# minio/minlz

Hardware: AMD Instinct MI355X
Metric: MB/s encode+decode, 8MB blocks L1 (higher is better)
Workload: dtype u8; 1 GPU; enwik8-like synthetic text (the reference's L1 compresses it to ~0.47; enwik8 itself is not available offline), 100000000 B per GPU in 8 MiB blocks (12 blocks), level 1, far=1; step = encode all blocks + decode all blocks, HBM-resident; block_size=8388608, bytes_per_gpu=100000000, ranks=1, backend=none (single process), device=AMD Radeon Graphics (gfx950:sramecc+:xnack-)

## Files before the change

minlz_amd/csrc/mlz_encode.hip.inc:

```

namespace mlz {

constexpr uint32_t kLaneCap = 32;
#ifndef MLZ_FAR_BITS
#define MLZ_FAR_BITS 17
#endif
#ifndef MLZ_EPOCH_LOG
#define MLZ_EPOCH_LOG 21
#endif
constexpr int kFarBits = MLZ_FAR_BITS;
constexpr int kEpochLog = MLZ_EPOCH_LOG;
static_assert((1u << kEpochLog) <= kMaxCopy3Offset, "a position's own epoch lies within one copy3 offset");
constexpr int kFarStride = 4;
#ifndef MLZ_SMALL_FB_SHIFT
#define MLZ_SMALL_FB_SHIFT 2
#endif
__host__ __device__ __forceinline__ constexpr int small_far_bits(uint64_t block_len) {
    int lg = 14 + MLZ_SMALL_FB_SHIFT;
    while (lg < 17 + MLZ_SMALL_FB_SHIFT && (1ull << lg) < block_len) lg++;
    return lg - MLZ_SMALL_FB_SHIFT;
}
constexpr uint32_t kFarMin = 8;
constexpr int kLevels = 4;

__device__ __forceinline__ uint64_t ld64u(const uint8_t* p) {
    uint64_t v;
    __builtin_memcpy(&v, p, 8);
    return v;
}
constexpr int kFarTagBits = 9;
constexpr uint32_t kFarTagMask = (1u << kFarTagBits) - 1;
struct FarHash { uint32_t idx, tag; };
__device__ __forceinline__ FarHash far_hash(uint64_t v, int bits, uint32_t tagmask = kFarTagMask) {
    const uint32_t a = (uint32_t(v) * 0x9E3779B1u + uint32_t(v >> 32)) * 0x85EBCA77u;
    return {a >> (32 - bits), (a >> (32 - bits - kFarTagBits)) & tagmask};
}
__device__ __forceinline__ uint32_t ctz64(uint64_t v) { return __builtin_ctzll(v); }
__device__ __forceinline__ uint64_t ballot64(bool p) { return __ballot(p); }
__device__ __forceinline__ uint32_t rdlane(uint32_t v, int l) { return __builtin_amdgcn_readlane(v, l); }
__device__ __forceinline__ uint32_t rdfirst(uint32_t v) { return __builtin_amdgcn_readfirstlane(v); }

constexpr uint32_t kPatternFast = 0xE4E4E4E4u;
#ifndef MLZ_PATTERN_DENSE
#define MLZ_PATTERN_DENSE 0xEEE7B9E4u
#endif
constexpr uint32_t kPatternDense = MLZ_PATTERN_DENSE;
#ifndef MLZ_PATTERN_THREE
#define MLZ_PATTERN_THREE 0xA9A9A994u
#endif
constexpr uint32_t kPatternThree = MLZ_PATTERN_THREE;
constexpr uint32_t kPatternFree = 0u;
__host__ __device__ __forceinline__ int tile_level_p(uint32_t tile_in_block, uint32_t pattern) { return int((pattern >> (2 * (tile_in_block & 15))) & 3); }
__host__ __device__ __forceinline__ int tile_level(uint32_t tile_in_block) { return tile_level_p(tile_in_block, kPatternFast); }
__host__ __device__ __forceinline__ uint32_t level_pattern_of(int level) { return level >= 2 ? kPatternDense : kPatternThree; }

__host__ __device__ __forceinline__ uint32_t far_sets(uint32_t pattern) { return pattern == kPatternFree ? 1u : uint32_t(kLevels - 1); }

__device__ __forceinline__ uint32_t match_len(const uint8_t* a, const uint8_t* b, uint32_t max) {
    uint32_t n = 0;
    while (n + 8 <= max) {
        uint64_t d = ld64u(a + n) ^ ld64u(b + n);
        if (d) return n + (ctz64(d) >> 3);
        n += 8;
    }
    while (n < max && a[n] == b[n]) n++;
    return n;
}

constexpr int kFarSliceBits = 15;
constexpr int kL2FarBitsBig = 18;
__host__ __device__ constexpr uint32_t far_tag_mask(int FB) { return FB == kL2FarBitsBig ? 0x1E0u : kFarTagMask; }
constexpr uint32_t far_slices(int fb) { return 1u << (fb - kFarSliceBits); }
constexpr uint64_t kBigBlock = 1u << 20;
template <int FB, int ST>
__global__ __launch_bounds__(1024) void far_build_kernel(const uint8_t* __restrict__ src_base, const BlockInfo* __restrict__ blocks,
                                                         uint32_t* __restrict__ far_tab, uint32_t epochs_per_block, uint32_t pattern,
                                                         uint32_t tab_log, uint32_t cls) {
    extern __shared__ __attribute__((aligned(16))) uint8_t smem[];
    uint32_t* slot = reinterpret_cast<uint32_t*>(smem);
    const uint32_t slice = blockIdx.x;
    const uint32_t ep = blockIdx.y;
    const BlockInfo b = blocks[blockIdx.z];
    if (cls != 2 && uint32_t(b.src_len >= kBigBlock) != cls) return;
    if (b.src_len > kMaxBlockSize) return;
    const int fb = FB ? FB : small_far_bits(b.src_len) + (ST == 2 ? 1 : 0);
    const uint32_t tlog = FB ? uint32_t(FB) : tab_log;
    const int sbits = fb < kFarSliceBits ? fb : kFarSliceBits;
    if (slice >= (1u << (fb - sbits))) return;
    const uint8_t* s = src_base + b.src_off;
    const int tid = threadIdx.x;
    for (uint32_t i = tid; i < (1u << sbits) / 4; i += 1024) reinterpret_cast<uint4*>(slot)[i] = uint4{0xffffffffu, 0xffffffffu, 0xffffffffu, 0xffffffffu};
    __syncthreads();
    const uint64_t e0 = uint64_t(ep) << kEpochLog;
    const uint64_t e1 = e0 + (1ull << kEpochLog) < b.src_len ? e0 + (1ull << kEpochLog) : b.src_len;
    constexpr uint32_t kPerTile = kTile / ST / 1024;
    constexpr int kFbTiles = ST >= 4 ? 2 : 1;
    constexpr uint32_t kBatch = kFbTiles * kPerTile;
    const uint32_t tiles_in_epoch = e1 > e0 && b.src_len >= 8 ? uint32_t((e1 - e0 + kTile - 1) >> kTileLog) : 0;
    constexpr uint32_t kEpochTiles = 1u << (kEpochLog - kTileLog);
    static_assert(kEpochTiles % 64 == 0, "an epoch is a whole number of 64-tile groups (4 periods of the level pattern each)");
    uint32_t need = 0;
    const bool free_levels = pattern == kPatternFree;
    {
        const uint64_t nt = (b.src_len + kTile - 1) >> kTileLog;
        for (uint32_t k = 1; k < 16 && k < nt; k++) need = need > uint32_t(tile_level_p(k, pattern)) ? need : uint32_t(tile_level_p(k, pattern));
        if (free_levels) need = nt > 1 ? 1 : 0;
    }
    for (uint32_t lset = 0; lset < need; lset++) {
      for (uint32_t g64 = 0; g64 < kEpochTiles; g64 += 64) {
        const uint32_t left = tiles_in_epoch > g64 ? tiles_in_epoch - g64 : 0;
        const uint64_t in_epoch = left >= 64 ? ~0ull : ((1ull << left) - 1);
        uint64_t todo = 0;
        for (uint32_t k = 0; k < 16; k++)
            if (free_levels || uint32_t(tile_level_p(k, pattern)) == lset) todo |= 0x0001000100010001ull << k;
        todo &= in_epoch;
        while (todo) {
            uint32_t kk[kFbTiles];
#pragma unroll
            for (int t = 0; t < kFbTiles; t++) { kk[t] = todo ? g64 + uint32_t(ctz64(todo)) : tiles_in_epoch; todo &= todo - 1; }
            uint64_t w[kBatch];
            uint64_t qq[kBatch];
            bool ok[kBatch];
#pragma unroll
            for (uint32_t u = 0; u < kBatch; u++) {
                const uint32_t k = kk[u / kPerTile];
                const uint64_t q = e0 + (uint64_t(k) << kTileLog) + (uint64_t(u % kPerTile) * 1024 + tid) * ST;
                qq[u] = q;
                ok[u] = k < tiles_in_epoch && q + 8 <= b.src_len && q < e1;
                w[u] = ld64u(s + (ok[u] ? q : 0));
            }
#pragma unroll
            for (uint32_t u = 0; u < kBatch; u++) {
                const FarHash fh = far_hash(w[u], fb, far_tag_mask(FB));
                if (ok[u] && (fh.idx >> sbits) == slice)
                    atomicMin(&slot[fh.idx & ((1u << sbits) - 1)], (uint32_t(qq[u]) << kFarTagBits) | fh.tag);
            }
        }
      }
        __syncthreads();
        const size_t tab = ((size_t(blockIdx.z) * far_sets(pattern) + lset) * epochs_per_block + ep) << tlog;
        uint32_t* out = far_tab + tab + (size_t(slice) << sbits);
        for (uint32_t i = tid; i < (1u << sbits) / 4; i += 1024) reinterpret_cast<uint4*>(out)[i] = reinterpret_cast<const uint4*>(slot)[i];
        __syncthreads();
    }
}

__device__ __forceinline__ uint32_t wave_incl_scan_u32(uint32_t v);
constexpr int kBinSliceBits = 14;
template <int FB, int ST> struct FarBin {
    static_assert(FB == kL2FarBitsBig, "the sorted word: 4 tag bits << 28 | window << 14 | bucket");
    static constexpr uint32_t kPerUnit = kTile / 2 / ST;
    static constexpr uint32_t kSlices = 1u << (FB - kBinSliceBits);
    static constexpr uint32_t kOffs = kSlices + 1;
    static constexpr uint32_t kCounters = 4 * kSlices * 64;
    static constexpr uint32_t kLds = kPerUnit * 4 + kCounters * 4 + kOffs * 4 + 64;
};
template <int FB, int ST>
__global__ __launch_bounds__(256) void far_bin_kernel(const uint8_t* __restrict__ src_base, const BlockInfo* __restrict__ blocks,
                                                      const uint32_t* __restrict__ tile_block, uint32_t* __restrict__ bins,
                                                      uint32_t* __restrict__ binoff) {
    using C = FarBin<FB, ST>;
    constexpr uint32_t kPerUnit = C::kPerUnit, kPerWave = kPerUnit / 4, kRounds = kPerWave / 64, kS = C::kSlices;
    static_assert(kPerUnit <= (1u << 14) && kRounds <= 64 && kRounds % 16 == 0, "window index in 14 bits; a lane's words in registers");
    extern __shared__ __attribute__((aligned(16))) uint8_t smem[];
    uint32_t* B = reinterpret_cast<uint32_t*>(smem);
    uint32_t* cnt = B + kPerUnit;
    uint32_t* segoff = cnt + C::kCounters;
    uint32_t* wsum = segoff + C::kOffs;
    const uint32_t unit = blockIdx.x, gt = unit >> 1;
    const BlockInfo b = blocks[tile_block[gt]];
    if (b.src_len < kBigBlock) return;
    const uint32_t tib = gt - b.first_tile;
    const uint64_t base = (uint64_t(tib) << kTileLog) + (unit & 1) * (kTile / 2);
    const uint8_t* s = src_base + b.src_off;
    const int tid = threadIdx.x, lane = tid & 63;
    const uint32_t wv = rdfirst(uint32_t(tid) >> 6);
    for (uint32_t i = tid; i < C::kCounters / 4; i += 256) reinterpret_cast<uint4*>(cnt)[i] = uint4{0, 0, 0, 0};
    __syncthreads();
    uint32_t word[kRounds];
    uint8_t tag4[kRounds];
    uint32_t* mine = cnt + wv * 64 + lane;
#pragma unroll
    for (uint32_t r0 = 0; r0 < kRounds; r0 += 16) {
        uint64_t w[16];
        bool ok[16];
#pragma unroll
        for (int u = 0; u < 16; u++) {
            const uint64_t q = base + uint64_t(wv * kPerWave + (r0 + u) * 64 + lane) * ST;
            ok[u] = q + 8 <= b.src_len;
            w[u] = ld64u(s + (ok[u] ? q : 0));
        }
#pragma unroll
        for (int u = 0; u < 16; u++) {
            const FarHash fh = far_hash(w[u], FB, far_tag_mask(FB));
            const uint32_t j = wv * kPerWave + (r0 + u) * 64 + lane;
            word[r0 + u] = ok[u] ? (fh.idx >> kBinSliceBits) << 28 | j << kBinSliceBits | (fh.idx & ((1u << kBinSliceBits) - 1)) : 0xffffffffu;
            tag4[r0 + u] = uint8_t(fh.tag >> 5);
            if (ok[u]) atomicAdd(&mine[(fh.idx >> kBinSliceBits) * 256], 1u);
        }
    }
    __syncthreads();
    {
        uint32_t v[16], sum = 0;
#pragma unroll
        for (int i = 0; i < 16; i++) { v[i] = cnt[tid * 16 + i]; sum += v[i]; }
        const uint32_t incl = wave_incl_scan_u32(sum);
        if (lane == 63) wsum[wv] = incl;
        __syncthreads();
        uint32_t carry = 0;
#pragma unroll
        for (uint32_t k = 0; k < 4; k++) carry += k < wv ? wsum[k] : 0;
        uint32_t run = carry + incl - sum;
#pragma unroll
        for (int i = 0; i < 16; i++) { cnt[tid * 16 + i] = run; run += v[i]; }
        if (tid == 255) segoff[kS] = run;
        __syncthreads();
        if (tid < int(kS)) segoff[tid] = cnt[tid * 256];
    }
#pragma unroll
    for (uint32_t r = 0; r < kRounds; r++)
        if (word[r] != 0xffffffffu) B[atomicAdd(&mine[(word[r] >> 28) * 256], 1u)] = (word[r] & 0x0fffffffu) | uint32_t(tag4[r]) << 28;
    __syncthreads();
    const uint32_t total = segoff[kS];
    uint32_t* out = bins + size_t(unit) * kPerUnit;
    for (uint32_t i = tid * 4; i < total; i += 1024) reinterpret_cast<uint4*>(out + i)[0] = reinterpret_cast<const uint4*>(B + i)[0];
    if (tid < int(C::kOffs)) binoff[size_t(unit) * C::kOffs + tid] = segoff[tid];
}

template <int FB, int ST>
__global__ __launch_bounds__(1024) void far_slice_kernel(const BlockInfo* __restrict__ blocks, const uint32_t* __restrict__ bins,
                                                         const uint32_t* __restrict__ binoff, uint32_t* __restrict__ far_tab, uint32_t epochs_per_block) {
    using C = FarBin<FB, ST>;
    constexpr uint32_t kPerUnit = C::kPerUnit, kSlice = 1u << kBinSliceBits;
    constexpr uint32_t kEpochUnits = 2u << (kEpochLog - kTileLog);
    static_assert(kEpochUnits == 128, "128 half tiles per epoch: a thread pair per unit for the segment offsets");
    extern __shared__ __attribute__((aligned(16))) uint8_t smem[];
    uint32_t* slot = reinterpret_cast<uint32_t*>(smem);
    uint32_t* so = slot + kSlice;
    const uint32_t slice = blockIdx.x, ep = blockIdx.y;
    const BlockInfo b = blocks[blockIdx.z];
    if (b.src_len < kBigBlock || b.n_tiles == 0) return;
    const uint32_t units_len = uint32_t((b.src_len + kTile / 2 - 1) / (kTile / 2));
    const uint32_t units = units_len < 2 * b.n_tiles ? units_len : 2 * b.n_tiles;
    const uint32_t u0 = ep * kEpochUnits, u1 = u0 + kEpochUnits < units ? u0 + kEpochUnits : units;
    if (u0 >= u1) return;
    const uint32_t nu = u1 - u0;
    const size_t unit0 = size_t(b.first_tile) * 2 + u0;
    const int tid = threadIdx.x;
    if (tid < 256) {
        const uint32_t u = uint32_t(tid) >> 1;
        so[tid] = u < nu ? binoff[(unit0 + u) * C::kOffs + slice + (tid & 1)] : 0u;
    }
    for (uint32_t i = tid; i < kSlice / 4; i += 1024) reinterpret_cast<uint4*>(slot)[i] = uint4{0xffffffffu, 0xffffffffu, 0xffffffffu, 0xffffffffu};
    __syncthreads();
    uint32_t* pre = so + 256;
    if (tid < 64) {
        const uint32_t a0 = so[4 * tid + 1] - so[4 * tid], a1 = so[4 * tid + 3] - so[4 * tid + 2];
        const uint32_t incl = wave_incl_scan_u32(a0 + a1);
        pre[2 * tid] = incl - a0 - a1; pre[2 * tid + 1] = incl - a1;
        if (tid == 63) pre[128] = incl;
    }
    __syncthreads();
    const uint32_t total = pre[128];
    for (uint32_t e0 = 0; e0 < total; e0 += 16 * 1024) {
        uint32_t w[16], ub[16];
#pragma unroll
        for (uint32_t k = 0; k < 16; k++) {
            const uint32_t e = e0 + 1024 * k + uint32_t(tid);
            const uint32_t ee = e < total ? e : total - 1;
            uint32_t u = 0;
#pragma unroll
            for (uint32_t step = 64; step; step >>= 1) u += pre[u + step] <= ee ? step : 0;
            ub[k] = e < total ? (u0 + u) * (kTile / 2) : 0xffffffffu;
            w[k] = bins[(unit0 + u) * kPerUnit + so[2 * u] + (ee - pre[u])];
        }
#pragma unroll
        for (uint32_t k = 0; k < 16; k++)
            if (ub[k] != 0xffffffffu)
                atomicMin(&slot[w[k] & (kSlice - 1)], (ub[k] + ((w[k] >> kBinSliceBits) & (kSlice - 1)) * ST) << kFarTagBits | (w[k] >> 28) << 5);
    }
    __syncthreads();
    uint32_t* tab = far_tab + ((size_t(blockIdx.z) * far_sets(kPatternFree) * epochs_per_block + ep) << FB) + (size_t(slice) << kBinSliceBits);
    for (uint32_t i = tid; i < kSlice / 4; i += 1024) reinterpret_cast<uint4*>(tab)[i] = reinterpret_cast<const uint4*>(slot)[i];
}

__device__ __forceinline__ uint64_t lds_ld64(const uint32_t* w, uint32_t p) {
    const uint32_t i = p >> 2, sh = p & 3;
    const uint32_t a = w[i], b = w[i + 1], c = w[i + 2];
    const uint32_t lo = __builtin_amdgcn_alignbyte(b, a, sh);
    const uint32_t hi = __builtin_amdgcn_alignbyte(c, b, sh);
    return lo | (uint64_t(hi) << 32);
}
__device__ __forceinline__ uint8_t lds_ld8(const uint32_t* w, uint32_t p) { return reinterpret_cast<const uint8_t*>(w)[p]; }
// ... 183 lines not shown
```

minlz_amd/csrc/mlz_hip.hip:

```cpp
#include <hip/hip_runtime.h>

#include <algorithm>
#include <atomic>
#include <condition_variable>
#include <cstdio>
#include <cstring>
#include <mutex>
#include <string>
#include <thread>
#include <type_traits>
#include <vector>

#include "../../include/minlz_hip.h"
#include "../../include/minlz_hip_search_batch.h"
#include "../../include/minlz_hip_search_batch_prune.h"
#include "../../include/minlz_hip_stream_set.h"
#include "../../include/minlz_hip_search_compressed.h"
#include "../../include/minlz_hip_search_compress.h"
#include "../../include/minlz_hip_sidecar_extract.h"
#include "../../include/minlz_hip_record_index_store.h"
#include "../../include/minlz_hip_encode_batch_tables.h"
#include "mlz_format.h"
#include "mlz_kernels.h"

// ... 165 lines not shown
        ev_res[id]++;
    }
};

namespace {

#define HIPCHK(ctx, call)                                                                 \
    do {                                                                                  \
        hipError_t e_ = (call);                                                           \
        if (e_ != hipSuccess) {                                                           \
            (ctx)->err = std::string(#call) + ": " + hipGetErrorString(e_);               \
            return -MLZ_ERR_HIP;                                                          \
        }                                                                                 \
    } while (0)

struct Timer {
    mlz_ctx* c; int id; hipStream_t s;
    bool on;
    Timer(mlz_ctx* c_, int id_, hipStream_t s_) : c(c_), id(id_), s(s_), on(c_->timing != 0 && ((c_->timer_mask >> id_) & 1) != 0) {
        if (!on) return;
        if (c->ev_last_call[id] != c->call_seq) {
            c->ev_last_call[id] = c->call_seq;
            if (c->timing == 1) {
                while (c->ev_res[id] < c->ev_cnt[id]) c->resolve_one(id);
                c->acc_ms[id] = 0; c->ev_calls[id] = 0;
            }
            c->ev_calls[id]++;
        }
        while (c->ev_cnt[id] - c->ev_res[id] >= uint64_t(mlz_ctx::kTimerRing)) c->resolve_one(id);
        (void)hipEventRecord(c->evr[id][c->ev_cnt[id] % mlz_ctx::kTimerRing][0], s);
    }
    ~Timer() {
        if (!on) return;
        (void)hipEventRecord(c->evr[id][c->ev_cnt[id] % mlz_ctx::kTimerRing][1], s);
        c->ev_cnt[id]++;
    }
};

struct WorkspaceOrder {
    mlz_ctx* c; hipStream_t s;
    WorkspaceOrder(mlz_ctx* c_, hipStream_t s_) : c(c_), s(s_) {
        if (c->ws_used && (c->ws_recorded || c->ws_stream != s)) {
            if (c->ws_recorded) (void)hipStreamWaitEvent(s, c->ws_done, 0);
            else if (hipEventRecord(c->ws_done, c->ws_stream) == hipSuccess) (void)hipStreamWaitEvent(s, c->ws_done, 0);
            else { (void)hipGetLastError(); (void)hipDeviceSynchronize(); }
        }
    }
    ~WorkspaceOrder() {
        c->ws_stream = s;
        c->ws_used = true;
        c->ws_recorded = false;
    }
};

int upload_blocks(mlz_ctx* c, hipStream_t st, const mlz_block_desc* desc, int n, bool tiles_from_dst, uint32_t* total_tiles, uint32_t* total_segs = nullptr,
                  const uint64_t* mirror = nullptr, bool any_length = false ) {
    c->dk = tiles_from_dst ? 1 : 0;
    std::vector<BlockInfo>& prev = c->h_blocks_prev_k[c->dk];
    c->h_blocks.resize(n);
    uint32_t tiles = 0, segs = 0;
    for (int i = 0; i < n; i++) {
        BlockInfo& b = c->h_blocks[i];
        b.src_off = desc[i].src_off; b.src_len = desc[i].src_len; b.dst_off = desc[i].dst_off; b.dst_cap = desc[i].dst_cap;
        b.mirror = mirror ? mirror[i] : 0;
        uint64_t span = tiles_from_dst ? desc[i].dst_cap : desc[i].src_len;
        if (span > kMaxBlockSize && !any_length) span = tiles_from_dst ? kMaxBlockSize : 0;
        b.first_tile = tiles;
        b.n_tiles = uint32_t((span + kTile - 1) >> kTileLog);
        tiles += b.n_tiles;
        b.first_seg = segs;
        b.n_segs = 0;
        if (tiles_from_dst) {
            uint64_t cl = std::min<uint64_t>(desc[i].src_len, 2 * std::min<uint64_t>(desc[i].dst_cap, kMaxBlockSize) + 32);
            b.n_segs = uint32_t((cl + kSeg - 1) >> kSegLog);
            segs += b.n_segs;
        }
    }
    *total_tiles = tiles;
    if (total_segs) *total_segs = segs;
    const bool same = prev.size() == c->h_blocks.size() && std::memcmp(prev.data(), c->h_blocks.data(), sizeof(BlockInfo) * n) == 0;
    if (same) return 0;
    c->h_tile_block.resize(tiles);
    c->h_seg_block.resize(segs);
    for (int i = 0; i < n; i++) {
        for (uint32_t t = 0; t < c->h_blocks[i].n_tiles; t++) c->h_tile_block[c->h_blocks[i].first_tile + t] = uint32_t(i);
        for (uint32_t t = 0; t < c->h_blocks[i].n_segs; t++) c->h_seg_block[c->h_blocks[i].first_seg + t] = uint32_t(i);
    }
    const size_t nb = sizeof(BlockInfo) * n, nt = sizeof(uint32_t) * tiles, ns = sizeof(uint32_t) * segs;
    const int sl = (c->up_slot ^= 1);
    if (c->upload_pending_k[sl]) { HIPCHK(c, hipEventSynchronize(c->upload_done_k[sl])); c->upload_pending_k[sl] = false; }
    if (nb + nt + ns > c->pinned_cap_k[sl]) {
        if (c->pinned_k[sl]) HIPCHK(c, hipHostFree(c->pinned_k[sl]));
        c->pinned_k[sl] = nullptr;
        c->pinned_cap_k[sl] = (nb + nt + ns) * 2 + 4096;
        HIPCHK(c, hipHostMalloc(&c->pinned_k[sl], c->pinned_cap_k[sl], hipHostMallocDefault));
    }
    char* pin = static_cast<char*>(c->pinned_k[sl]);
    HIPCHK(c, c->d_blocks_cur().ensure(nb + 64));
    HIPCHK(c, c->d_tile_block_cur().ensure(nt + 64));
    HIPCHK(c, c->d_seg_block_cur().ensure(ns + 64));
    std::memcpy(pin, c->h_blocks.data(), nb);
    std::memcpy(pin + nb, c->h_tile_block.data(), nt);
    std::memcpy(pin + nb + nt, c->h_seg_block.data(), ns);
    if (nb) HIPCHK(c, hipMemcpyAsync(c->d_blocks_cur().p, pin, nb, hipMemcpyHostToDevice, st));
    if (nt) HIPCHK(c, hipMemcpyAsync(c->d_tile_block_cur().p, pin + nb, nt, hipMemcpyHostToDevice, st));
    if (ns) HIPCHK(c, hipMemcpyAsync(c->d_seg_block_cur().p, pin + nb + nt, ns, hipMemcpyHostToDevice, st));
    HIPCHK(c, hipEventRecord(c->upload_done_k[sl], st));
    c->upload_pending_k[sl] = true;
    prev = c->h_blocks;
    return 0;
}

template <class F> int for_each_group(mlz_ctx* c, const mlz_block_desc* desc, int n, bool by_dst, F fn) {
    int b0 = 0;
    while (b0 < n) {
        uint64_t bytes = 0;
        int b1 = b0;
        while (b1 < n) {
            const uint64_t span = std::min<uint64_t>(by_dst ? desc[b1].dst_cap : desc[b1].src_len, kMaxBlockSize);
            if (b1 > b0 && bytes + span > c->device_group) break;
            bytes += span;
            b1++;
        }
        const int r = fn(b0, b1 - b0);
        if (r) return r;
        b0 = b1;
    }
    return 0;
}

template <class List> int raise_lds_once(mlz_ctx* c, bool& raised, const List& list) {
    if (raised) return 0;
    for (const auto& k : list) HIPCHK(c, hipFuncSetAttribute(reinterpret_cast<const void*>(k.fn), hipFuncAttributeMaxDynamicSharedMemorySize, int(k.lds)));
    raised = true;
    return 0;
}
template <class Fn> struct Kernel { Fn fn; uint32_t lds; };
struct AnyKernel : Kernel<const void*> { template <class F> AnyKernel(F* f, uint32_t l) : Kernel{reinterpret_cast<const void*>(f), l} {} };
using Kernels = std::initializer_list<AnyKernel>;

using MatchFn = void (*)(const uint8_t*, const BlockInfo*, const uint32_t*, uint2*, uint32_t*, const uint32_t*, uint32_t, uint32_t, uint32_t, uint32_t, uint32_t,
                         uint32_t, uint8_t*, uint32_t*);
enum MatchId { M_L1_BIG_FAR, M_L1_SMALL_FAR, M_L1_BIG, M_L1_SMALL, M_SUPERFAST, M_L2_BIG, M_L2_SMALL, M_L2_ONE_TILE, M_COUNT };
const Kernel<MatchFn> kMatch[M_COUNT] = {
    {match_tiles_kernel<true, MLZ_M2_NW, kM2HashBitsBig, kFarBits, false>, M2Cfg<kM2HashBitsBig>::kLds},
    {match_tiles_kernel<true, MLZ_M2_NW, kM2HashBitsSmall, 0, false>, M2Cfg<kM2HashBitsSmall>::kLds},
    {match_tiles_kernel<false, MLZ_M2_NW, kM2HashBitsBig, kFarBits, false>, M2Cfg<kM2HashBitsBig>::kLds},
    {match_tiles_kernel<false, MLZ_M2_NW, kM2HashBitsSmall, kFarBits, false>, M2Cfg<kM2HashBitsSmall>::kLds},
    {match_tiles_kernel<false, MLZ_M2_NW, kM2HashBitsSuperFast, kFarBits, false>, M2Cfg<kM2HashBitsSuperFast>::kLds},
    {match_tiles_kernel<true, MLZ_M2_NW, kM2HashBitsSmall, kL2FarBits, true>, M2Cfg<kM2HashBitsSmall>::kLds},
    {match_tiles_kernel<true, MLZ_M2_NW, kM2HashBitsSmall, 0, true>, M2Cfg<kM2HashBitsSmall>::kLds},
    {match_tiles_kernel<false, MLZ_M2_NW, kM2HashBitsSmall, kL2FarBits, true>, M2Cfg<kM2HashBitsSmall>::kLds},
};
using FarBuildFn = void (*)(const uint8_t*, const BlockInfo*, uint32_t*, uint32_t, uint32_t, uint32_t, uint32_t);
const Kernel<FarBuildFn> kFarBuild[4] = {
    {far_build_kernel<0, kFarStride>, 4u << kFarSliceBits}, {far_build_kernel<kFarBits, kFarStride>, 4u << kFarSliceBits},
    {far_build_kernel<0, kL2FarStride>, 4u << kFarSliceBits}, {far_build_kernel<kL2FarBits, kL2FarStride>, 4u << kFarSliceBits},
};

struct MatchPlan { int n; struct { MatchId id; uint32_t cls; } launch[2]; };
MatchPlan match_plan(int level, bool far, bool any_big, bool any_small) {
    if (level == MLZ_LEVEL_SUPERFAST) return {1, {{M_SUPERFAST, 2u}}};
    const bool l2 = level == MLZ_LEVEL_BALANCED;
    if (l2 && !far) return {1, {{M_L2_ONE_TILE, 2u}}};
    MatchPlan p{};
    if (any_big) p.launch[p.n++] = {l2 ? M_L2_BIG : far ? M_L1_BIG_FAR : M_L1_BIG, any_small ? 1u : 2u};
    if (any_small) p.launch[p.n++] = {l2 ? M_L2_SMALL : far ? M_L1_SMALL_FAR : M_L1_SMALL, any_big ? 0u : 2u};
    return p;
}

struct EncGroup {
    int level, n;
    const BlockInfo* blocks; const uint32_t* tile_block;
    uint32_t tiles, epochs, pattern, far_gap;
    size_t units;
    bool far, any_big, any_small;
    int fbits;
};

int encode_far_tables(mlz_ctx* c, hipStream_t st, const EncGroup& g, const uint8_t* d_src, const mlz_block_desc* desc) {
    Timer t(c, T_FAR, st);
    const bool l2 = g.level == MLZ_LEVEL_BALANCED;
    HIPCHK(c, c->d_far.ensure(((size_t(g.n) * far_sets(g.pattern) * g.epochs) << g.fbits) * 4));
    if (int r = raise_lds_once(c, c->far_attr, kFarBuild)) return r;
    auto build = [&](const Kernel<FarBuildFn>& v, dim3 grid, uint32_t lds, uint32_t cls) {
        hipLaunchKernelGGL(v.fn, grid, dim3(1024), lds, st, d_src, g.blocks, c->d_far.as<uint32_t>(), g.epochs, g.pattern, uint32_t(g.fbits), cls);
    };
    if (g.any_big) {
        if (l2 && g.pattern == kPatternFree && !c->far_slices_l2) {
            using FBn = FarBin<kL2FarBits, kL2FarStride>;
            const size_t units2 = size_t(g.tiles) * 2;
            HIPCHK(c, c->d_farbin.ensure(units2 * FBn::kPerUnit * 4 + units2 * FBn::kOffs * 4 + 256));
            uint32_t* bins = c->d_farbin.as<uint32_t>();
            uint32_t* binoff = bins + units2 * FBn::kPerUnit;
            constexpr uint32_t kSliceLds = (4u << kBinSliceBits) + 256 * 4 + 132 * 4;
            if (int r = raise_lds_once(c, c->farbin_attr, Kernels{{far_bin_kernel<kL2FarBits, kL2FarStride>, FBn::kLds}, {far_slice_kernel<kL2FarBits, kL2FarStride>, kSliceLds}})) return r;
            hipLaunchKernelGGL((far_bin_kernel<kL2FarBits, kL2FarStride>), dim3(uint32_t(units2)), dim3(256), FBn::kLds, st, d_src, g.blocks, g.tile_block, bins, binoff);
            hipLaunchKernelGGL((far_slice_kernel<kL2FarBits, kL2FarStride>), dim3(FBn::kSlices, g.epochs, g.n), dim3(1024), kSliceLds, st, g.blocks, bins, binoff, c->d_far.as<uint32_t>(), g.epochs);
        } else
            build(kFarBuild[2 * l2 + 1], dim3(far_slices(l2 ? kL2FarBits : kFarBits), g.epochs, g.n), kFarBuild[2 * l2 + 1].lds, g.any_small ? 1u : 2u);
    }
    if (g.any_small) {
        uint64_t max_small = 0;
        for (int i = 0; i < g.n; i++) if (desc[i].src_len < kBigBlock) max_small = std::max<uint64_t>(max_small, desc[i].src_len);
        const int sb = small_far_bits(max_small) + (l2 ? 1 : 0);
        const uint32_t lds = 4u << std::min<int>(sb, kFarSliceBits);
        build(kFarBuild[2 * l2], dim3(1u << (std::max<int>(sb, kFarSliceBits) - kFarSliceBits), 1, g.n), lds, g.any_big ? 0u : 2u);
    }
    return 0;
}

int encode_match(mlz_ctx* c, hipStream_t st, const EncGroup& g, const uint8_t* d_src) {
    HIPCHK(c, c->d_recs.ensure(g.units * kRecPerPiece * sizeof(uint2)));
    HIPCHK(c, c->d_piece_cnt.ensure(g.units * sizeof(uint32_t)));
    if (int r = raise_lds_once(c, c->enc_attrs, kMatch)) return r;
    const uint32_t* ftab = g.far ? c->d_far.as<uint32_t>() : nullptr;
    uint8_t* fuse_scratch = c->fuse_ser ? c->d_scratch.as<uint8_t>() : nullptr;
    {
        Timer t(c, T_ENC_TILES, st);
        const uint32_t grid = ((g.tiles + 7) / 8) * 8;
        const MatchPlan plan = match_plan(g.level, g.far, g.any_big, g.any_small);
        for (int i = 0; i < plan.n; i++) {
            const Kernel<MatchFn>& v = kMatch[plan.launch[i].id];
            hipLaunchKernelGGL(v.fn, dim3(grid), dim3(256), v.lds, st, d_src, g.blocks, g.tile_block, c->d_recs.as<uint2>(), c->d_piece_cnt.as<uint32_t>(), ftab, g.epochs,
                               g.pattern, g.tiles, plan.launch[i].cls, uint32_t(g.fbits), g.far_gap, fuse_scratch, c->d_tile_size.as<uint32_t>());
        }
    }
    if (!fuse_scratch) {
        Timer t(c, T_ENC_SER, st);
        hipLaunchKernelGGL(serialize_pieces_kernel, dim3(g.tiles), dim3(256), kSerLds, st, d_src, g.blocks, g.tile_block, c->d_recs.as<uint2>(),
                           c->d_piece_cnt.as<uint32_t>(), c->d_scratch.as<uint8_t>(), c->d_tile_size.as<uint32_t>());
    }
    return 0;
}

void encode_layout_gather(mlz_ctx* c, hipStream_t st, const EncGroup& g, const uint8_t* d_src, uint8_t* d_dst, const mlz_block_desc* desc, int64_t* d_out_len,
                          bool with_header) {
    bool fold = c->fold_layout && g.tiles > 0 && g.level != MLZ_LEVEL_UNCOMPRESSED;
    for (int i = 0; fold && i < g.n; i++) {
        const uint64_t len = desc[i].src_len;
        if (len == 0 || len > kMaxBlockSize || desc[i].dst_cap < (with_header ? len + 2 : len)) fold = false;
    }
    if (!fold) {
        Timer t(c, T_ENC_LAYOUT, st);
        hipLaunchKernelGGL(encode_layout_kernel, dim3(g.n), dim3(64), 0, st, g.blocks, c->d_tile_size.as<uint32_t>(), c->d_tile_out.as<uint32_t>(), d_dst, d_out_len,
                           c->d_flags.as<uint32_t>(), g.level, with_header ? 1 : 0, kSubLog);
    }
    if (g.tiles > 0) {
        Timer t(c, T_ENC_GATHER, st);
        const auto gather = fold ? encode_gather2_kernel<true> : encode_gather2_kernel<false>;
        hipLaunchKernelGGL(gather, dim3(g.tiles), dim3(256), 0, st, d_src, g.blocks, g.tile_block, c->d_scratch.as<uint8_t>(),
                           c->d_tile_size.as<uint32_t>(), c->d_tile_out.as<uint32_t>(), d_dst, c->d_flags.as<uint32_t>(), with_header ? 1 : 0, g.level, d_out_len);
    }
}

int encode_device_group(mlz_ctx* c, hipStream_t st, int level, const uint8_t* d_src, uint8_t* d_dst, const mlz_block_desc* desc, int n,
                        int64_t* d_out_len, bool with_header, const uint64_t* mirror) {
    EncGroup g{level, n};
    int r = upload_blocks(c, st, desc, n, false, &g.tiles, nullptr, mirror);
    if (r) return r;
    g.blocks = c->d_blocks_cur().as<BlockInfo>(); g.tile_block = c->d_tile_block_cur().as<uint32_t>();
    g.units = size_t(g.tiles) << kSubLog;
    HIPCHK(c, c->d_tile_size.ensure(sizeof(uint32_t) * (g.units + 1)));
    HIPCHK(c, c->d_tile_out.ensure(sizeof(uint32_t) * (g.units + 1)));
    HIPCHK(c, c->d_flags.ensure(sizeof(uint32_t) * n));
    if (level != MLZ_LEVEL_UNCOMPRESSED && g.tiles > 0) {
        HIPCHK(c, c->d_scratch.ensure(g.units * kPieceScratch));
        const bool l2 = level == MLZ_LEVEL_BALANCED;
        uint64_t maxlen = 0;
        for (int i = 0; i < n; i++) {
            const uint64_t len = std::min<uint64_t>(desc[i].src_len, kMaxBlockSize);
            maxlen = std::max(maxlen, len);
            (len >= kM2BigBlock ? g.any_big : g.any_small) = true;
        }
        g.epochs = uint32_t((maxlen + (1u << kEpochLog) - 1) >> kEpochLog);
        g.far = ((c->encode_far && level != MLZ_LEVEL_SUPERFAST) || l2) && maxlen > kTile;
        g.pattern = (l2 && c->l2_free) ? kPatternFree : level_pattern_of(level);
        g.fbits = g.any_big ? (l2 ? kL2FarBits : kFarBits) : small_far_bits(maxlen) + (l2 ? 1 : 0);
        g.far_gap = g.pattern == kPatternFree && l2 ? uint32_t(c->l2_gap - 1) << kTileLog : 0u;
        if (g.far) r = encode_far_tables(c, st, g, d_src, desc);
        if (!r) r = encode_match(c, st, g, d_src);
        if (r) return r;
    }
    encode_layout_gather(c, st, g, d_src, d_dst, desc, d_out_len, with_header);
    HIPCHK(c, hipGetLastError());
    return 0;
}

uint32_t gen_settle_wgs(mlz_ctx* c, int n) {
    const uint32_t grid = c->gen_grid > 0 ? uint32_t(c->gen_grid) : uint32_t(c->n_cus);
    const uint32_t cap = c->gen_settle_cap > 0 ? uint32_t(c->gen_settle_cap) : grid / 4;
    return std::max<uint32_t>(4u, std::min<uint32_t>(4u * uint32_t(n), cap) & ~3u);
}

int decode_parallel(mlz_ctx* c, hipStream_t st, const uint8_t* d_src, uint8_t* d_dst, const mlz_block_desc* desc, int n, int64_t* d_out_len,
                    bool raw_body, const uint64_t* mirror) {
    uint32_t tiles = 0, segs = 0;
    int r = upload_blocks(c, st, desc, n, true, &tiles, &segs, mirror);
    if (r) return r;
    constexpr size_t kAl = 256;
    Carve cv;
    const auto r_dec = cv.take<DecBlock>(size_t(n), kAl);
    const auto r_exit = cv.take<uint32_t>(size_t(segs) * kExitKeep, kAl);
    const auto r_rexit = cv.take<uint8_t>(size_t(segs) * kSeg, kAl);
    const auto r_entry = cv.take<uint32_t>(segs, kAl);
    const auto r_tstart = cv.take<TileStart>(tiles, kAl);
    const auto r_tpos = cv.take<uint32_t>(size_t(segs) * kSeg, kAl);
    const auto r_rd = cv.take<uint32_t>(size_t(segs) * kSegThreads, kAl), r_rr = cv.take<uint32_t>(size_t(segs) * kSegThreads, kAl);
    const auto r_order = cv.take<uint32_t>(tiles, kAl), r_glist = cv.take<uint32_t>(size_t(n), kAl);
    const auto r_xcnt = cv.take<GenTile>(tiles, kAl);
    const size_t zero_begin = cv.take<uint32_t>(0, kAl).off;
    const auto r_done = cv.take<uint32_t>(tiles, kAl), r_ticket = cv.take<uint32_t>(kAl / 4, kAl);
    const auto r_gen = cv.take<GenCtl>(1, kAl);
    const auto r_sstate = cv.take<unsigned long long>(size_t(segs) * 4, kAl);
    const auto r_sviol = cv.take<uint8_t>(size_t(segs) * 4, kAl);
    const size_t zero_end = cv.take<uint32_t>(0, kAl).off;
    const auto r_tok16 = cv.take<uint16_t>(size_t(segs) * kSeg, kAl);
    HIPCHK(c, c->d_dec.ensure(cv.take<uint8_t>(0, kAl).off));
    void* ws = c->d_dec.p;
    DecBlock* dec = r_dec.at(ws);
    TileStart* tile_start = r_tstart.at(ws);
    uint8_t *rexit_tab = r_rexit.at(ws), *sviol = r_sviol.at(ws);
    uint32_t *exit_tab = r_exit.at(ws), *seg_entry = r_entry.at(ws), *tok_pos = r_tpos.at(ws), *round_d = r_rd.at(ws), *round_rep = r_rr.at(ws), *order = r_order.at(ws);
    uint32_t *tile_done = r_done.at(ws), *ticket = r_ticket.at(ws);
    GenCtl* gen = r_gen.at(ws);
    uint32_t* gen_words = reinterpret_cast<uint32_t*>(gen);
    unsigned long long* sstate = r_sstate.at(ws);
    uint16_t* tok16 = r_tok16.at(ws);
    Carve idx;
    const auto r_gmap = idx.take<uint16_t>(size_t(tiles) << kTileLog);
    const auto r_gpool = idx.take<uint8_t>(size_t(tiles) << kTileLog);
    const auto r_ext = idx.take<ExtEnt>((size_t(segs) << kSegLog) + size_t(tiles) * kExtPerTile + 64 * size_t(n));
    bool jump = c->general_algo == 0 && c->decode_algo == 0 && tiles > 0;
    if (jump && c->d_idx.ensure(idx.bytes + 256) != hipSuccess) {
        (void)hipGetLastError();
        c->gen_fallbacks++;
        jump = false;
    }
    uint32_t* gen_list = jump ? r_glist.at(ws) : nullptr;
    const BlockInfo* blocks = c->d_blocks_cur().as<BlockInfo>();
    const uint32_t* tile_block = c->d_tile_block_cur().as<uint32_t>();
    const uint32_t* seg_block = c->d_seg_block_cur().as<uint32_t>();
    if ((r = raise_lds_once(c, c->dec_attrs, Kernels{{dec_exit_kernel, kExitLds}, {dec_index1_kernel, kIdxLds}, {dec_exec2_kernel, kExecLds}}))) return r;
    L0Cands cands;
    uint32_t n_cand = 0;
    bool l0 = tiles && c->level0_by_e && c->decode_algo == 0 && uint64_t(n) < (1ull << kL0BlockBits);
    if (l0) {
        const uint32_t cap = std::min<uint32_t>(c->l0_grid_cap > 0 ? uint32_t(c->l0_grid_cap) : uint32_t(c->n_cus), kL0MaxCands);
        for (int i = 0; i < n && n_cand <= cap; i++)
            for (uint32_t j = 0; 16 * j < c->h_blocks[i].n_tiles && n_cand <= cap; j++, n_cand++)
                if (n_cand < cap) cands.e[n_cand] = uint32_t(i) | (j << kL0BlockBits);
        l0 = n_cand >= 1 && n_cand <= cap;
    }
    if (l0 && !c->l0_attr) {
        if (!c->l0_attr_failed && hipFuncSetAttribute(reinterpret_cast<const void*>(dec_level0_kernel), hipFuncAttributeMaxDynamicSharedMemorySize, int(kGenLds)) == hipSuccess) c->l0_attr = true;
        else { (void)hipGetLastError(); c->l0_attr_failed = true; l0 = false; }
    }
    uint32_t* n_general = jump ? &gen->n_general : nullptr;
    HIPCHK(c, c->d_gen_acc.ensure(64));
    const uint32_t acc_reset = c->acc_call != c->dec_call ? 1u : 0u;
// ... 715 lines not shown
```

Measured before the change: 75670 MB/s.

## Remap far-build grid for L2 slice locality and load 16-byte windows per thread

```diff
diff --git a/minlz_amd/csrc/mlz_encode.hip.inc b/minlz_amd/csrc/mlz_encode.hip.inc
--- a/minlz_amd/csrc/mlz_encode.hip.inc
+++ b/minlz_amd/csrc/mlz_encode.hip.inc
@@ -70,17 +70,26 @@
 constexpr int kFarSliceBits = 15;
 constexpr int kL2FarBitsBig = 18;
 __host__ __device__ constexpr uint32_t far_tag_mask(int FB) { return FB == kL2FarBitsBig ? 0x1E0u : kFarTagMask; }
-constexpr uint32_t far_slices(int fb) { return 1u << (fb - kFarSliceBits); }
 constexpr uint64_t kBigBlock = 1u << 20;
+struct FarPlace { uint32_t slice, group; };
+__host__ __device__ __forceinline__ FarPlace far_place(uint32_t wg, uint32_t slice_log) {
+    const uint32_t r = wg >> 3;
+    return {r & ((1u << slice_log) - 1), ((r >> slice_log) << 3) | (wg & 7)};
+}
+__host__ __device__ __forceinline__ uint32_t far_grid(uint32_t n_groups, uint32_t slice_log) { return ((n_groups + 7) / 8 * 8) << slice_log; }
 template <int FB, int ST>
 __global__ __launch_bounds__(1024) void far_build_kernel(const uint8_t* __restrict__ src_base, const BlockInfo* __restrict__ blocks,
                                                          uint32_t* __restrict__ far_tab, uint32_t epochs_per_block, uint32_t pattern,
-                                                         uint32_t tab_log, uint32_t cls) {
+                                                         uint32_t tab_log, uint32_t cls, uint32_t slice_log, uint32_t grid_epochs,
+                                                         uint32_t n_groups) {
     extern __shared__ __attribute__((aligned(16))) uint8_t smem[];
     uint32_t* slot = reinterpret_cast<uint32_t*>(smem);
-    const uint32_t slice = blockIdx.x;
-    const uint32_t ep = blockIdx.y;
-    const BlockInfo b = blocks[blockIdx.z];
+    const FarPlace at = far_place(blockIdx.x, slice_log);
+    if (at.group >= n_groups) return;
+    const uint32_t slice = at.slice;
+    const uint32_t blk = at.group / grid_epochs;
+    const uint32_t ep = at.group % grid_epochs;
+    const BlockInfo b = blocks[blk];
     if (cls != 2 && uint32_t(b.src_len >= kBigBlock) != cls) return;
     if (b.src_len > kMaxBlockSize) return;
     const int fb = FB ? FB : small_far_bits(b.src_len) + (ST == 2 ? 1 : 0);
@@ -118,27 +127,58 @@
             uint32_t kk[kFbTiles];
 #pragma unroll
             for (int t = 0; t < kFbTiles; t++) { kk[t] = todo ? g64 + uint32_t(ctz64(todo)) : tiles_in_epoch; todo &= todo - 1; }
-            uint64_t w[kBatch];
-            uint64_t qq[kBatch];
-            bool ok[kBatch];
-#pragma unroll
-            for (uint32_t u = 0; u < kBatch; u++) {
-                const uint32_t k = kk[u / kPerTile];
-                const uint64_t q = e0 + (uint64_t(k) << kTileLog) + (uint64_t(u % kPerTile) * 1024 + tid) * ST;
-                qq[u] = q;
-                ok[u] = k < tiles_in_epoch && q + 8 <= b.src_len && q < e1;
-                w[u] = ld64u(s + (ok[u] ? q : 0));
-            }
-#pragma unroll
-            for (uint32_t u = 0; u < kBatch; u++) {
-                const FarHash fh = far_hash(w[u], fb, far_tag_mask(FB));
-                if (ok[u] && (fh.idx >> sbits) == slice)
-                    atomicMin(&slot[fh.idx & ((1u << sbits) - 1)], (uint32_t(qq[u]) << kFarTagBits) | fh.tag);
+            bool whole = true;
+#pragma unroll
+            for (int t = 0; t < kFbTiles; t++) whole = whole && kk[t] < tiles_in_epoch && e0 + (uint64_t(kk[t] + 1) << kTileLog) + 8 <= b.src_len;
+            if (whole) {
+                constexpr uint32_t kWin = 16 / ST;
+                constexpr uint32_t kGroups = kPerTile / kWin;
+                constexpr uint32_t kG = kFbTiles * kGroups;
+                constexpr uint32_t kX = ST == 4 ? 1 : 2;
+                static_assert(ST == 2 || ST == 4, "windows start on even bytes of a group");
+                static_assert((kWin - 1) * ST + 8 <= 16 + 4 * kX && 4 * kX <= 8, "the last window ends inside the loaded bytes, those inside the tile's 8 spare bytes");
+                uint32_t at[kG];
+                uint32_t d[kG][4 + kX];
+#pragma unroll
+                for (uint32_t g = 0; g < kG; g++) at[g] = uint32_t(e0) + (kk[g / kGroups] << kTileLog) + ((g % kGroups) * 1024 + uint32_t(tid)) * 16;
+#pragma unroll
+                for (uint32_t g = 0; g < kG; g++) __builtin_memcpy(d[g], s + at[g], 16 + 4 * kX);
+#pragma unroll
+                for (uint32_t g = 0; g < kG; g++) {
+#pragma unroll
+                    for (uint32_t j = 0; j < kWin; j++) {
+                        const uint32_t o = j * ST;
+                        const auto dword_at = [&](uint32_t i) {
+                            if constexpr (ST == 4) return d[g][i / 4];
+                            else return i % 4 ? (d[g][i / 4] >> 16) | (d[g][i / 4 + 1] << 16) : d[g][i / 4];
+                        };
+                        const FarHash fh = far_hash(uint64_t(dword_at(o + 4)) << 32 | dword_at(o), fb, far_tag_mask(FB));
+                        if ((fh.idx >> sbits) == slice) atomicMin(&slot[fh.idx & ((1u << sbits) - 1)], ((at[g] + o) << kFarTagBits) | fh.tag);
+                    }
+                }
+            } else {
+                uint64_t w[kBatch];
+                uint64_t qq[kBatch];
+                bool ok[kBatch];
+#pragma unroll
+                for (uint32_t u = 0; u < kBatch; u++) {
+                    const uint32_t k = kk[u / kPerTile];
+                    const uint64_t q = e0 + (uint64_t(k) << kTileLog) + (uint64_t(u % kPerTile) * 1024 + tid) * ST;
+                    qq[u] = q;
+                    ok[u] = k < tiles_in_epoch && q + 8 <= b.src_len && q < e1;
+                    w[u] = ld64u(s + (ok[u] ? q : 0));
+                }
+#pragma unroll
+                for (uint32_t u = 0; u < kBatch; u++) {
+                    const FarHash fh = far_hash(w[u], fb, far_tag_mask(FB));
+                    if (ok[u] && (fh.idx >> sbits) == slice)
+                        atomicMin(&slot[fh.idx & ((1u << sbits) - 1)], (uint32_t(qq[u]) << kFarTagBits) | fh.tag);
+                }
             }
         }
       }
         __syncthreads();
-        const size_t tab = ((size_t(blockIdx.z) * far_sets(pattern) + lset) * epochs_per_block + ep) << tlog;
+        const size_t tab = ((size_t(blk) * far_sets(pattern) + lset) * epochs_per_block + ep) << tlog;
         uint32_t* out = far_tab + tab + (size_t(slice) << sbits);
         for (uint32_t i = tid; i < (1u << sbits) / 4; i += 1024) reinterpret_cast<uint4*>(out)[i] = reinterpret_cast<const uint4*>(slot)[i];
         __syncthreads();
diff --git a/minlz_amd/csrc/mlz_hip.hip b/minlz_amd/csrc/mlz_hip.hip
--- a/minlz_amd/csrc/mlz_hip.hip
+++ b/minlz_amd/csrc/mlz_hip.hip
@@ -341,7 +341,7 @@
     {match_tiles_kernel<true, MLZ_M2_NW, kM2HashBitsSmall, 0, true>, M2Cfg<kM2HashBitsSmall>::kLds},
     {match_tiles_kernel<false, MLZ_M2_NW, kM2HashBitsSmall, kL2FarBits, true>, M2Cfg<kM2HashBitsSmall>::kLds},
 };
-using FarBuildFn = void (*)(const uint8_t*, const BlockInfo*, uint32_t*, uint32_t, uint32_t, uint32_t, uint32_t);
+using FarBuildFn = void (*)(const uint8_t*, const BlockInfo*, uint32_t*, uint32_t, uint32_t, uint32_t, uint32_t, uint32_t, uint32_t, uint32_t);
 const Kernel<FarBuildFn> kFarBuild[4] = {
     {far_build_kernel<0, kFarStride>, 4u << kFarSliceBits}, {far_build_kernel<kFarBits, kFarStride>, 4u << kFarSliceBits},
     {far_build_kernel<0, kL2FarStride>, 4u << kFarSliceBits}, {far_build_kernel<kL2FarBits, kL2FarStride>, 4u << kFarSliceBits},
@@ -372,8 +372,10 @@
     const bool l2 = g.level == MLZ_LEVEL_BALANCED;
     HIPCHK(c, c->d_far.ensure(((size_t(g.n) * far_sets(g.pattern) * g.epochs) << g.fbits) * 4));
     if (int r = raise_lds_once(c, c->far_attr, kFarBuild)) return r;
-    auto build = [&](const Kernel<FarBuildFn>& v, dim3 grid, uint32_t lds, uint32_t cls) {
-        hipLaunchKernelGGL(v.fn, grid, dim3(1024), lds, st, d_src, g.blocks, c->d_far.as<uint32_t>(), g.epochs, g.pattern, uint32_t(g.fbits), cls);
+    auto build = [&](const Kernel<FarBuildFn>& v, uint32_t slice_log, uint32_t grid_epochs, uint32_t lds, uint32_t cls) {
+        const uint32_t groups = uint32_t(g.n) * grid_epochs;
+        hipLaunchKernelGGL(v.fn, dim3(far_grid(groups, slice_log)), dim3(1024), lds, st, d_src, g.blocks, c->d_far.as<uint32_t>(), g.epochs, g.pattern, uint32_t(g.fbits), cls,
+                           slice_log, grid_epochs, groups);
     };
     if (g.any_big) {
         if (l2 && g.pattern == kPatternFree && !c->far_slices_l2) {
@@ -387,14 +389,14 @@
             hipLaunchKernelGGL((far_bin_kernel<kL2FarBits, kL2FarStride>), dim3(uint32_t(units2)), dim3(256), FBn::kLds, st, d_src, g.blocks, g.tile_block, bins, binoff);
             hipLaunchKernelGGL((far_slice_kernel<kL2FarBits, kL2FarStride>), dim3(FBn::kSlices, g.epochs, g.n), dim3(1024), kSliceLds, st, g.blocks, bins, binoff, c->d_far.as<uint32_t>(), g.epochs);
         } else
-            build(kFarBuild[2 * l2 + 1], dim3(far_slices(l2 ? kL2FarBits : kFarBits), g.epochs, g.n), kFarBuild[2 * l2 + 1].lds, g.any_small ? 1u : 2u);
+            build(kFarBuild[2 * l2 + 1], uint32_t((l2 ? kL2FarBits : kFarBits) - kFarSliceBits), g.epochs, kFarBuild[2 * l2 + 1].lds, g.any_small ? 1u : 2u);
     }
     if (g.any_small) {
         uint64_t max_small = 0;
         for (int i = 0; i < g.n; i++) if (desc[i].src_len < kBigBlock) max_small = std::max<uint64_t>(max_small, desc[i].src_len);
         const int sb = small_far_bits(max_small) + (l2 ? 1 : 0);
         const uint32_t lds = 4u << std::min<int>(sb, kFarSliceBits);
-        build(kFarBuild[2 * l2], dim3(1u << (std::max<int>(sb, kFarSliceBits) - kFarSliceBits), 1, g.n), lds, g.any_big ? 0u : 2u);
+        build(kFarBuild[2 * l2], uint32_t(std::max<int>(sb, kFarSliceBits) - kFarSliceBits), 1, lds, g.any_big ? 0u : 2u);
     }
     return 0;
 }
```

Result: faster. 76680 MB/s (median of 6 runs) (+1.3%).
